# matt-graham/mici

Hardware: NVIDIA H100
Metric: leapfrog steps/sec (aggregate over chains) (higher is better)
Workload: dtype f64

## Files before the change

mici_b200/csrc/leapfrog_dmma.cuh:

```cuda
#pragma once
#include <cfloat>
#include <type_traits>

#include "targets.cuh"

namespace mb200 {

__device__ __forceinline__ void dmma_m8n8k4(double& c0, double& c1, double a, double b) {
  asm volatile(
      "mma.sync.aligned.m8n8k4.row.col.f64.f64.f64.f64 {%0,%1}, {%2}, {%3}, {%0,%1};\n"
      : "+d"(c0), "+d"(c1)
      : "d"(a), "d"(b));
}

__device__ __forceinline__ void dmma_m16n8k16(double& c0, double& c1, double& c2, double& c3,
                                              const double2 (&a)[2][2], const double2 (&b)[2]) {
  asm volatile(
      "mma.sync.aligned.m16n8k16.row.col.f64.f64.f64.f64 {%0,%1,%2,%3}, "
      "{%4,%5,%6,%7,%8,%9,%10,%11}, {%12,%13,%14,%15}, {%0,%1,%2,%3};\n"
      : "+d"(c0), "+d"(c1), "+d"(c2), "+d"(c3)
      : "d"(a[0][0].x), "d"(a[1][0].x), "d"(a[0][0].y), "d"(a[1][0].y),
        "d"(a[0][1].x), "d"(a[1][1].x), "d"(a[0][1].y), "d"(a[1][1].y),
        "d"(b[0].x), "d"(b[0].y), "d"(b[1].x), "d"(b[1].y));
}

__device__ __forceinline__ uint32_t smem_u32(const void* p) {
  return static_cast<uint32_t>(__cvta_generic_to_shared(p));
}

__device__ __forceinline__ void named_barrier_sync(int id, int nthreads) {
  asm volatile("bar.sync %0, %1;" ::"r"(id), "r"(nthreads) : "memory");
}

#ifndef MB200_K1_TRACE
#define MB200_K1_TRACE(phase)
#endif
#ifndef MB200_K1_TRACE_AFTER
#define MB200_K1_TRACE_AFTER(phase, x)
#endif
#ifndef MB200_K1_MARK
#define MB200_K1_MARK(id)
#endif

constexpr int DMMA_TILES_PER_CTA = 8;
#ifndef MB200_DMMA_GROUPS
#define MB200_DMMA_GROUPS 4
#endif
constexpr int DMMA_GROUPS = MB200_DMMA_GROUPS;
__host__ __device__ constexpr int dmma_tile_count(int g) {
  return DMMA_TILES_PER_CTA / DMMA_GROUPS + (g < DMMA_TILES_PER_CTA % DMMA_GROUPS ? 1 : 0);
}
__host__ __device__ constexpr int dmma_tile_start(int g) {
  return g * (DMMA_TILES_PER_CTA / DMMA_GROUPS) +
         (g < DMMA_TILES_PER_CTA % DMMA_GROUPS ? g : DMMA_TILES_PER_CTA % DMMA_GROUPS);
}
constexpr int DMMA_MAX_MT = (DMMA_TILES_PER_CTA + DMMA_GROUPS - 1) / DMMA_GROUPS;
constexpr int DMMA_THREADS = 32 * 4 * DMMA_GROUPS;
constexpr int DMMA_ROWS_PER_CTA = 8 * DMMA_TILES_PER_CTA;

template <int DP>
struct DmmaSmem {
  static constexpr int LDA = DP + 8;
  double A[DP * LDA];
  double P[DMMA_ROWS_PER_CTA * LDA];
  double psum[DMMA_ROWS_PER_CTA][4];
  double rscal[DMMA_ROWS_PER_CTA];
  double ex[2][DMMA_ROWS_PER_CTA][4];
  unsigned long long mbar;
};

template <class Target, int DP, int MT, bool PC>
__device__ __forceinline__ void leapfrog_dmma_group(
    DmmaSmem<DP>& sm, const Target& target, const double* q_in, const double* p_in,
    double* q_out, double* p_out, const int32_t* __restrict__ dir,
    const double* __restrict__ step_sizes, int64_t n_chains, int dim,
    double step_size, int n_steps, double* __restrict__ h_out, int32_t* __restrict__ status,
    int32_t* __restrict__ n_done, int64_t chain0, int row0, int w, int lane, int bar_id,
    int cta_threads, bool vec2, int32_t* __restrict__ counters) {
  constexpr int LDA = DmmaSmem<DP>::LDA;
  constexpr int NT = DP / 32;
  constexpr int KS = DP / 4;
  const int r = lane >> 2, c = lane & 3;
  const int col0 = w * (DP / 4);
  const double mh = -0.5 * step_size;
  const bool owner = (w == 0) && (c == 0);

  double q[MT][NT][2], mhr[PC ? MT : 1];
  bool live[MT];
  int row[MT];
  auto load_scale = [&](int64_t ch) {
    const double d = (dir != nullptr && dir[ch] < 0) ? -1.0 : 1.0;
    return PC ? d * step_sizes[ch] : d;
  };
  const uint32_t pofs = (uint32_t)((row0 + r) * LDA + col0 + 2 * c);
  auto pslot = [&](int mt, int nt) -> double2& {
    return *reinterpret_cast<double2*>(&sm.P[pofs + mt * 8 * LDA + 8 * nt]);
  };

#pragma unroll
  for (int mt = 0; mt < MT; ++mt) {
    row[mt] = row0 + 8 * mt + r;
    const int64_t ch = chain0 + row[mt];
    live[mt] = ch < n_chains;
    const double sgn = live[mt] ? load_scale(ch) : (PC ? 0.0 : 1.0);
    if (PC) mhr[mt] = -0.5 * (sgn * sgn);
#pragma unroll
    for (int nt = 0; nt < NT; ++nt) {
      const int i = col0 + 8 * nt + 2 * c;
      double2 a = make_double2(0.0, 0.0), b = make_double2(0.0, 0.0);
      if (live[mt] && i < dim) {
        if (vec2) {
          a = *reinterpret_cast<const double2*>(q_in + (size_t)ch * dim + i);
          b = *reinterpret_cast<const double2*>(p_in + (size_t)ch * dim + i);
        } else {
          a.x = q_in[(size_t)ch * dim + i], b.x = p_in[(size_t)ch * dim + i];
          if (i + 1 < dim) a.y = q_in[(size_t)ch * dim + i + 1], b.y = p_in[(size_t)ch * dim + i + 1];
        }
      }
      q[mt][nt][0] = a.x, q[mt][nt][1] = a.y;
      pslot(mt, nt) = make_double2(sgn * b.x, sgn * b.y);
    }
  }

  int s = -1;

  auto tile_sums = [&]() {
    if (!Target::TILE_SUM) return;
    double v[MT];
#pragma unroll
    for (int mt = 0; mt < MT; ++mt) {
      double t0 = q[mt][0][0] * q[mt][0][0];
      if (Target::COORD0) t0 = owner ? 0.0 : t0;
      t0 = fma(q[mt][0][1], q[mt][0][1], t0);
      if (mt == 0) MB200_K1_TRACE_AFTER(6, t0);
      double t1 = 0.0;
#pragma unroll
      for (int nt = 1; nt < NT; ++nt) {
        double& t = (nt & 1) ? t1 : t0;
        t = fma(q[mt][nt][0], q[mt][nt][0], t);
        t = fma(q[mt][nt][1], q[mt][nt][1], t);
      }
      v[mt] = t0 + t1;
    }
#pragma unroll
    for (int mt = 0; mt < MT; ++mt) v[mt] += __shfl_xor_sync(FULL_MASK, v[mt], 1);
#pragma unroll
    for (int mt = 0; mt < MT; ++mt) v[mt] += __shfl_xor_sync(FULL_MASK, v[mt], 2);
#pragma unroll
    for (int mt = 0; mt < MT; ++mt)
      if (c == 0) sm.psum[row[mt]][w] = v[mt];
  };
  auto publish_partials = [&]() {
    if (Target::ROW_SCALAR && w == 0) {
      double v0 = (c == 0) ? q[0][0][0] : 0.0;
#pragma unroll
      for (int mt = 1; mt < MT; ++mt) {
        const double vm = __shfl_sync(FULL_MASK, q[mt][0][0], lane & ~3);
        v0 = (c == mt) ? vm : v0;
      }
      tile_sums();
      const double rs = target.row_scalar(v0);
      if (c < MT) sm.rscal[row0 + 8 * c + r] = rs;
    } else {
      tile_sums();
    }
  };

  auto update_phase = [&](auto kicks_tag) {
    constexpr int KICKS = decltype(kicks_tag)::value;
    double2 pv[MT][NT];
    if (KICKS > 0) {
#pragma unroll
      for (int mt = 0; mt < MT; ++mt)
#pragma unroll
        for (int nt = 0; nt < NT; ++nt) pv[mt][nt] = pslot(mt, nt);
    }
    publish_partials();
    MB200_K1_TRACE(2);
    named_barrier_sync(bar_id, 128);
    MB200_K1_TRACE(3);
    if (KICKS == 0) return;
    double rs[MT];
#pragma unroll
    for (int mt = 0; mt < MT; ++mt) rs[mt] = Target::ROW_SCALAR ? sm.rscal[row[mt]] : 1.0;
#pragma unroll
    for (int mt = 0; mt < MT; ++mt) {
      const double mhm = PC ? mhr[PC ? mt : 0] : mh;
      const double coef = target.kick_coef(mhm, rs[mt]);
      double c00 = coef, a00 = q[mt][0][0];
      if (Target::COORD0 && w == 0) {
        const double4 ps = *reinterpret_cast<const double4*>(&sm.psum[row[mt]][0]);
        const double g0 = target.grad0(q[mt][0][0], ((ps.x + ps.y) + ps.z) + ps.w, rs[mt]);
        c00 = owner ? mhm : coef;
        a00 = owner ? g0 : a00;
      }
#pragma unroll
      for (int nt = 0; nt < NT; ++nt) {
        double2 v = pv[mt][nt];
        if (Target::LINEAR) {
#pragma unroll
          for (int k = 0; k < KICKS; ++k) {
            v.x = (nt == 0) ? fma(c00, a00, v.x) : fma(coef, q[mt][nt][0], v.x);
            v.y = fma(coef, q[mt][nt][1], v.y);
          }
        } else {
#pragma unroll
          for (int k = 0; k < KICKS; ++k)
            target.kick_pair_nl(mhm, q[mt][nt][0], q[mt][nt][1], v.x, v.y);
        }
        pslot(mt, nt) = v;
      }
    }
    MB200_K1_TRACE(4);
    named_barrier_sync(bar_id, 128);
    MB200_K1_TRACE(5);
  };
  using K0 = std::integral_constant<int, 0>;
  using K1 = std::integral_constant<int, 1>;
  using K2 = std::integral_constant<int, 2>;

  auto drift = [&](double (&acc)[MT][NT][2]) {
    const double2* a_base = reinterpret_cast<const double2*>(&sm.P[(row0 + r) * LDA + 2 * c]);
    const double2* b_base = reinterpret_cast<const double2*>(&sm.A[(col0 + r) * LDA + 2 * c]);
    if constexpr (MT == 2) {
#pragma unroll 2
      for (int j = 0; j < KS / 4; ++j) {
        double2 a[2][2], b[NT][2];
#pragma unroll
        for (int mt = 0; mt < 2; ++mt)
#pragma unroll
          for (int h = 0; h < 2; ++h) a[mt][h] = a_base[mt * 4 * LDA + 4 * (2 * j + h)];
#pragma unroll
        for (int nt = 0; nt < NT; ++nt)
#pragma unroll
          for (int h = 0; h < 2; ++h) b[nt][h] = b_base[nt * 4 * LDA + 4 * (2 * j + h)];
#pragma unroll
        for (int nt = 0; nt < NT; ++nt)
          dmma_m16n8k16(acc[0][nt][0], acc[0][nt][1], acc[1][nt][0], acc[1][nt][1], a, b[nt]);
      }
    } else {
      constexpr bool KSPLIT = (MT == 1);
      double acc2[KSPLIT ? NT : 1][2];
      if (KSPLIT) {
#pragma unroll
        for (int nt = 0; nt < NT; ++nt) acc2[nt][0] = 0.0, acc2[nt][1] = 0.0;
      }
#pragma unroll 4
      for (int j = 0; j < KS / 2; ++j) {
        double2 a[MT], b[NT];
#pragma unroll
        for (int mt = 0; mt < MT; ++mt) a[mt] = a_base[mt * 4 * LDA + 4 * j];
#pragma unroll
        for (int nt = 0; nt < NT; ++nt) b[nt] = b_base[nt * 4 * LDA + 4 * j];
#pragma unroll
        for (int mt = 0; mt < MT; ++mt)
#pragma unroll
          for (int nt = 0; nt < NT; ++nt)
            dmma_m8n8k4(acc[mt][nt][0], acc[mt][nt][1], a[mt].x, b[nt].x);
#pragma unroll
        for (int mt = 0; mt < MT; ++mt)
#pragma unroll
          for (int nt = 0; nt < NT; ++nt) {
            if (KSPLIT) dmma_m8n8k4(acc2[nt][0], acc2[nt][1], a[mt].y, b[nt].y);
            else dmma_m8n8k4(acc[mt][nt][0], acc[mt][nt][1], a[mt].y, b[nt].y);
          }
      }
      if (KSPLIT) {
#pragma unroll
        for (int nt = 0; nt < NT; ++nt) acc[0][nt][0] += acc2[nt][0], acc[0][nt][1] += acc2[nt][1];
      }
    }
  };

  MB200_K1_MARK(4);
  if (n_steps > 0) update_phase(K1{});
  else update_phase(K0{});
  MB200_K1_MARK(5);
  for (s = 0; s < n_steps - 1; ++s) {
    MB200_K1_TRACE(0);
    drift(q);
    MB200_K1_TRACE(1);
    update_phase(K2{});
  }
  if (n_steps > 0) {
    drift(q);
    update_phase(K1{});
  }

  MB200_K1_MARK(6);
#pragma unroll
  for (int mt = 0; mt < MT; ++mt) {
    const int64_t ch = chain0 + row[mt];
    if (!live[mt]) continue;
    const double sgn = load_scale(ch);
#pragma unroll
    for (int nt = 0; nt < NT; ++nt) {
      const int i = col0 + 8 * nt + 2 * c;
      if (i < dim) {
        const double2 sv = pslot(mt, nt);
        double2 pv = make_double2(sgn * sv.x, sgn * sv.y);
        if (PC) {
          if (sgn != 0.0) {
            pv = make_double2(sv.x / sgn, sv.y / sgn);
          } else {
            pv.x = p_in[(size_t)ch * dim + i];
            pv.y = (i + 1 < dim) ? p_in[(size_t)ch * dim + i + 1] : 0.0;
          }
          if (h_out != nullptr && !(sgn * sgn >= DBL_MIN)) pslot(mt, nt) = pv;
        }
        if (vec2) {
          *reinterpret_cast<double2*>(q_out + (size_t)ch * dim + i) =
              make_double2(q[mt][nt][0], q[mt][nt][1]);
          *reinterpret_cast<double2*>(p_out + (size_t)ch * dim + i) = pv;
        } else {
          q_out[(size_t)ch * dim + i] = q[mt][nt][0], p_out[(size_t)ch * dim + i] = pv.x;
          if (i + 1 < dim)
            q_out[(size_t)ch * dim + i + 1] = q[mt][nt][1], p_out[(size_t)ch * dim + i + 1] = pv.y;
        }
      }
    }
    if (w == 0 && c == 0) {
      if (status != nullptr) status[ch] = MB200_STATUS_OK;
      if (n_done != nullptr) n_done[ch] = n_steps;
      if (counters != nullptr) counters[ch * MB200_N_COUNTERS + MB200_COUNT_GRAD] += n_steps + 1;
    }
  }

  MB200_K1_MARK(7);
  if (h_out != nullptr) {
    if (PC) named_barrier_sync(bar_id, 128);
    double l[MT], kin[MT], u[MT][NT][2];
#pragma unroll
    for (int mt = 0; mt < MT; ++mt) {
      double red[2] = {0.0, 1.0};
      if (Target::TILE_SUM) {
        const double4 ps = *reinterpret_cast<const double4*>(&sm.psum[row[mt]][0]);
        red[0] = ((ps.x + ps.y) + ps.z) + ps.w;
      }
      if (Target::ROW_SCALAR) red[1] = sm.rscal[row[mt]];
      l[mt] = 0.0;
#pragma unroll
      for (int nt = 0; nt < NT; ++nt) {
        const int i = col0 + 8 * nt + 2 * c;
        if (i < dim) l[mt] += target.nld_pair(i, q[mt][nt][0], q[mt][nt][1], red);
        u[mt][nt][0] = 0.0, u[mt][nt][1] = 0.0;
      }
    }
    drift(u);
#pragma unroll
    for (int mt = 0; mt < MT; ++mt) {
      kin[mt] = 0.0;
#pragma unroll
      for (int nt = 0; nt < NT; ++nt) {
        const double2 sv = pslot(mt, nt);
        kin[mt] = fma(sv.x, u[mt][nt][0], kin[mt]);
        kin[mt] = fma(sv.y, u[mt][nt][1], kin[mt]);
      }
      kin[mt] += __shfl_xor_sync(FULL_MASK, kin[mt], 1);
      kin[mt] += __shfl_xor_sync(FULL_MASK, kin[mt], 2);
      l[mt] += __shfl_xor_sync(FULL_MASK, l[mt], 1);
      l[mt] += __shfl_xor_sync(FULL_MASK, l[mt], 2);
      if (c == 0) {
        sm.ex[0][row[mt]][w] = kin[mt];
        sm.ex[1][row[mt]][w] = l[mt];
      }
    }
    named_barrier_sync(bar_id, 128);
    if (w == 0 && c == 0) {
#pragma unroll
      for (int mt = 0; mt < MT; ++mt) {
        if (!live[mt]) continue;
        const double4 k4 = *reinterpret_cast<const double4*>(&sm.ex[0][row[mt]][0]);
        const double4 l4 = *reinterpret_cast<const double4*>(&sm.ex[1][row[mt]][0]);
        const double ks = ((k4.x + k4.y) + k4.z) + k4.w;
        const double ls = ((l4.x + l4.y) + l4.z) + l4.w;
        if (PC) {
          const double e = step_sizes[chain0 + row[mt]];
          h_out[chain0 + row[mt]] = ls + 0.5 * (e * e >= DBL_MIN ? ks / (e * e) : ks);
        } else {
          h_out[chain0 + row[mt]] = ls + 0.5 * (ks / step_size);
        }
      }
    }
  }
}

template <class Target, int DP, bool PC>
__global__ void __launch_bounds__(DMMA_THREADS, 1)
    leapfrog_dmma_kernel(const double* q_in, const double* p_in, double* q_out, double* p_out,
                         const int32_t* __restrict__ dir, const double* __restrict__ step_sizes,
                         int64_t n_chains, int dim,
                         double step_size, int n_steps, const double* __restrict__ minv,
                         ModelArgs model, double* __restrict__ h_out,
                         int32_t* __restrict__ status, int32_t* __restrict__ n_done,
                         int tiles_per_cta, int vec2, int tma_rows) {
  extern __shared__ __align__(128) unsigned char smem_raw[];
  DmmaSmem<DP>& sm = *reinterpret_cast<DmmaSmem<DP>*>(smem_raw);
  constexpr int LDA = DmmaSmem<DP>::LDA;
  const int tid = threadIdx.x;
  const int lane = tid & 31;
  const int warp = tid >> 5;
  const int group = warp >> 2;
  const int w = ((warp & 3) + group) & 3;
  const Target target(model, dim);
  MB200_K1_MARK(0);

  const uint32_t mbar = smem_u32(&sm.mbar);
  if (tma_rows && warp == 0) {
    if (lane == 0) {
      asm volatile("mbarrier.init.shared::cta.b64 [%0], 1;" ::"r"(mbar));
      asm volatile("fence.mbarrier_init.release.cluster;" ::: "memory");
    }
    __syncwarp();
    const uint32_t row_bytes = (uint32_t)dim * 8u;
    if (lane == 0)
      asm volatile("mbarrier.arrive.expect_tx.shared::cta.b64 _, [%0], %1;" ::"r"(mbar),
                   "r"(row_bytes * (uint32_t)dim)
                   : "memory");
    __syncwarp();
#pragma unroll 1
    for (int row = lane; row < dim; row += 32) {
      const unsigned long long src =
          reinterpret_cast<unsigned long long>(minv) + (unsigned long long)row * row_bytes;
      asm volatile(
          "cp.async.bulk.shared::cluster.global.mbarrier::complete_tx::bytes [%0], [%1], %2, [%3];"
          ::"r"(smem_u32(&sm.A[row * LDA])),
          "l"(src), "r"(row_bytes), "r"(mbar)
          : "memory");
    }
  }
  {
    const int64_t chain0 = (int64_t)blockIdx.x * (8 * tiles_per_cta);
    const int64_t left = n_chains - chain0;
    const int64_t rows = left < 8 * tiles_per_cta ? left : 8 * tiles_per_cta;
    const int64_t lines = (rows * dim * 8 + 127) / 128;
    for (int64_t i = tid; i < 2 * lines; i += blockDim.x) {
      const double* base = (i < lines ? q_in : p_in) + (size_t)chain0 * dim;
      const char* ptr = reinterpret_cast<const char*>(base) + (i < lines ? i : i - lines) * 128;
      asm volatile("prefetch.global.L2 [%0];" ::"l"(ptr));
    }
  }
  if (!tma_rows) {
    for (int idx = tid; idx < dim * dim; idx += blockDim.x) {
      const int row = idx / dim, col = idx - row * dim;
      sm.A[row * LDA + col] = minv[idx];
    }
  }
  if (dim < DP) {
    for (int idx = tid; idx < DP * DP; idx += blockDim.x) {
      const int row = idx / DP, col = idx - row * DP;
      if (row >= dim || col >= dim) sm.A[row * LDA + col] = 0.0;
    }
  }
  MB200_K1_MARK(1);
  __syncthreads();
  if (tma_rows) {
    uint32_t done = 0;
    while (!done) {
      asm volatile(
          "{\n .reg .pred p;\n mbarrier.try_wait.parity.shared::cta.b64 p, [%1], 0;\n"
          " selp.u32 %0, 1, 0, p;\n}"
          : "=r"(done)
          : "r"(mbar)
          : "memory");
    }
  }
  MB200_K1_MARK(2);
  if (!PC)
#pragma unroll 4
  for (int idx = tid; idx < DP * (DP / 2); idx += blockDim.x) {
    const int row = idx / (DP / 2), c2 = idx - row * (DP / 2);
    double2* ptr = reinterpret_cast<double2*>(&sm.A[row * LDA]) + c2;
    double2 v = *ptr;
    v.x *= step_size, v.y *= step_size;
    *ptr = v;
  }
  __syncthreads();
  MB200_K1_MARK(3);

  const int rows_per_cta = 8 * tiles_per_cta;
  for (int64_t blk = blockIdx.x; blk * rows_per_cta < n_chains; blk += gridDim.x) {
    const int64_t chain0 = blk * rows_per_cta;
    const int64_t left = n_chains - chain0;
    const int tiles = (int)((left >= rows_per_cta) ? tiles_per_cta : (left + 7) / 8);
    const int base = tiles / DMMA_GROUPS, rem = tiles % DMMA_GROUPS;
    const int mt = base + (group < rem ? 1 : 0);
    const int row0 = 8 * (group * base + (group < rem ? group : rem));
    const int cta_threads = 128 * (tiles < DMMA_GROUPS ? tiles : DMMA_GROUPS);
#define MB200_GROUP(MT)                                                                       \
  leapfrog_dmma_group<Target, DP, MT, PC>(sm, target, q_in, p_in, q_out, p_out, dir,          \
                                          step_sizes, n_chains, dim, step_size, n_steps,      \
                                          h_out, status, n_done, chain0, row0, w, lane,       \
                                          1 + group, cta_threads, vec2 != 0, model.counters)
    if (DMMA_MAX_MT >= 4 && mt == 4) MB200_GROUP(4);
    else if (DMMA_MAX_MT >= 3 && mt == 3) MB200_GROUP(3);
    else if (mt == 2) MB200_GROUP(2);
    else if (mt == 1) MB200_GROUP(1);
#undef MB200_GROUP
    __syncthreads();
  }
}

}
```

Measured before the change: 1.443 billion.

## Split each DMMA row group across two warps with register-held momenta and pairwise barriers

Each row group now uses two warps, each owning half of the columns, instead of four warps owning quarters. Momenta stay in registers, and a warp's own half feeds the tensor-core drift directly. Only the half the partner needs is published to shared memory, signalled with bar.arrive and a per-warp named barrier. This removes the second barrier per step and lets each warp start on its own half while the partner is still publishing. It halves the CTA thread count and raises the register load per thread, which may cut occupancy and latency hiding.

```diff
diff --git a/mici_b200/csrc/leapfrog_dmma.cuh b/mici_b200/csrc/leapfrog_dmma.cuh
--- a/mici_b200/csrc/leapfrog_dmma.cuh
+++ b/mici_b200/csrc/leapfrog_dmma.cuh
@@ -32,6 +32,10 @@
   asm volatile("bar.sync %0, %1;" ::"r"(id), "r"(nthreads) : "memory");
 }
 
+__device__ __forceinline__ void named_barrier_arrive(int id, int nthreads) {
+  asm volatile("bar.arrive %0, %1;" ::"r"(id), "r"(nthreads) : "memory");
+}
+
 #ifndef MB200_K1_TRACE
 #define MB200_K1_TRACE(phase)
 #endif
@@ -43,19 +47,9 @@
 #endif
 
 constexpr int DMMA_TILES_PER_CTA = 8;
-#ifndef MB200_DMMA_GROUPS
-#define MB200_DMMA_GROUPS 4
-#endif
-constexpr int DMMA_GROUPS = MB200_DMMA_GROUPS;
-__host__ __device__ constexpr int dmma_tile_count(int g) {
-  return DMMA_TILES_PER_CTA / DMMA_GROUPS + (g < DMMA_TILES_PER_CTA % DMMA_GROUPS ? 1 : 0);
-}
-__host__ __device__ constexpr int dmma_tile_start(int g) {
-  return g * (DMMA_TILES_PER_CTA / DMMA_GROUPS) +
-         (g < DMMA_TILES_PER_CTA % DMMA_GROUPS ? g : DMMA_TILES_PER_CTA % DMMA_GROUPS);
-}
+constexpr int DMMA_GROUPS = 4;
 constexpr int DMMA_MAX_MT = (DMMA_TILES_PER_CTA + DMMA_GROUPS - 1) / DMMA_GROUPS;
-constexpr int DMMA_THREADS = 32 * 4 * DMMA_GROUPS;
+constexpr int DMMA_THREADS = 32 * 2 * DMMA_GROUPS;
 constexpr int DMMA_ROWS_PER_CTA = 8 * DMMA_TILES_PER_CTA;
 
 template <int DP>
@@ -75,17 +69,22 @@
     double* q_out, double* p_out, const int32_t* __restrict__ dir,
     const double* __restrict__ step_sizes, int64_t n_chains, int dim,
     double step_size, int n_steps, double* __restrict__ h_out, int32_t* __restrict__ status,
-    int32_t* __restrict__ n_done, int64_t chain0, int row0, int w, int lane, int bar_id,
-    int cta_threads, bool vec2, int32_t* __restrict__ counters) {
+    int32_t* __restrict__ n_done, int64_t chain0, int row0, int h, int lane, int group, bool vec2,
+    int32_t* __restrict__ counters) {
+  static_assert(MT == 1 || MT == 2, "a group owns one or two row tiles");
   constexpr int LDA = DmmaSmem<DP>::LDA;
-  constexpr int NT = DP / 32;
-  constexpr int KS = DP / 4;
+  constexpr int NT = DP / 16;
+  constexpr int NQ = NT / 2;
   const int r = lane >> 2, c = lane & 3;
-  const int col0 = w * (DP / 4);
+  const int col0 = h * (DP / 2);
+  const int bar_pair = 1 + group;
+  const int bar_own = 6 + 2 * group + h;
+  const int bar_partner = bar_own ^ 1;
   const double mh = -0.5 * step_size;
-  const bool owner = (w == 0) && (c == 0);
+  const bool owner = (h == 0) && (c == 0);
 
   double q[MT][NT][2], mhr[PC ? MT : 1];
+  double2 sv[MT][NT];
   bool live[MT];
   int row[MT];
   auto load_scale = [&](int64_t ch) {
@@ -118,7 +117,7 @@
         }
       }
       q[mt][nt][0] = a.x, q[mt][nt][1] = a.y;
-      pslot(mt, nt) = make_double2(sgn * b.x, sgn * b.y);
+      sv[mt][nt] = make_double2(sgn * b.x, sgn * b.y);
     }
   }
 
@@ -126,32 +125,40 @@
 
   auto tile_sums = [&]() {
     if (!Target::TILE_SUM) return;
-    double v[MT];
-#pragma unroll
-    for (int mt = 0; mt < MT; ++mt) {
-      double t0 = q[mt][0][0] * q[mt][0][0];
-      if (Target::COORD0) t0 = owner ? 0.0 : t0;
-      t0 = fma(q[mt][0][1], q[mt][0][1], t0);
-      if (mt == 0) MB200_K1_TRACE_AFTER(6, t0);
-      double t1 = 0.0;
-#pragma unroll
-      for (int nt = 1; nt < NT; ++nt) {
-        double& t = (nt & 1) ? t1 : t0;
-        t = fma(q[mt][nt][0], q[mt][nt][0], t);
-        t = fma(q[mt][nt][1], q[mt][nt][1], t);
-      }
-      v[mt] = t0 + t1;
-    }
-#pragma unroll
-    for (int mt = 0; mt < MT; ++mt) v[mt] += __shfl_xor_sync(FULL_MASK, v[mt], 1);
-#pragma unroll
-    for (int mt = 0; mt < MT; ++mt) v[mt] += __shfl_xor_sync(FULL_MASK, v[mt], 2);
+    double v[MT][2];
 #pragma unroll
     for (int mt = 0; mt < MT; ++mt)
-      if (c == 0) sm.psum[row[mt]][w] = v[mt];
+#pragma unroll
+      for (int qq = 0; qq < 2; ++qq) {
+        const int n0 = qq * NQ;
+        double t0 = q[mt][n0][0] * q[mt][n0][0];
+        if (Target::COORD0 && qq == 0) t0 = owner ? 0.0 : t0;
+        t0 = fma(q[mt][n0][1], q[mt][n0][1], t0);
+        if (mt == 0 && qq == 0) MB200_K1_TRACE_AFTER(6, t0);
+        double t1 = 0.0;
+#pragma unroll
+        for (int n = 1; n < NQ; ++n) {
+          double& t = (n & 1) ? t1 : t0;
+          t = fma(q[mt][n0 + n][0], q[mt][n0 + n][0], t);
+          t = fma(q[mt][n0 + n][1], q[mt][n0 + n][1], t);
+        }
+        v[mt][qq] = t0 + t1;
+      }
+#pragma unroll
+    for (int mt = 0; mt < MT; ++mt)
+#pragma unroll
+      for (int qq = 0; qq < 2; ++qq) v[mt][qq] += __shfl_xor_sync(FULL_MASK, v[mt][qq], 1);
+#pragma unroll
+    for (int mt = 0; mt < MT; ++mt)
+#pragma unroll
+      for (int qq = 0; qq < 2; ++qq) v[mt][qq] += __shfl_xor_sync(FULL_MASK, v[mt][qq], 2);
+#pragma unroll
+    for (int mt = 0; mt < MT; ++mt)
+      if (c == 0)
+        *reinterpret_cast<double2*>(&sm.psum[row[mt]][2 * h]) = make_double2(v[mt][0], v[mt][1]);
   };
   auto publish_partials = [&]() {
-    if (Target::ROW_SCALAR && w == 0) {
+    if (Target::ROW_SCALAR && h == 0) {
       double v0 = (c == 0) ? q[0][0][0] : 0.0;
 #pragma unroll
       for (int mt = 1; mt < MT; ++mt) {
@@ -166,125 +173,149 @@
     }
   };
 
-  auto update_phase = [&](auto kicks_tag) {
+  auto store_momenta = [&]() {
+#pragma unroll
+    for (int mt = 0; mt < MT; ++mt)
+#pragma unroll
+      for (int nt = 0; nt < NT; ++nt) pslot(mt, nt) = sv[mt][nt];
+    named_barrier_arrive(bar_own, 64);
+  };
+
+  auto update_phase = [&](auto kicks_tag, auto publish_tag) {
     constexpr int KICKS = decltype(kicks_tag)::value;
-    double2 pv[MT][NT];
-    if (KICKS > 0) {
-#pragma unroll
-      for (int mt = 0; mt < MT; ++mt)
-#pragma unroll
-        for (int nt = 0; nt < NT; ++nt) pv[mt][nt] = pslot(mt, nt);
-    }
+    constexpr bool PUBLISH = decltype(publish_tag)::value;
     publish_partials();
     MB200_K1_TRACE(2);
-    named_barrier_sync(bar_id, 128);
+    named_barrier_sync(bar_pair, 64);
     MB200_K1_TRACE(3);
-    if (KICKS == 0) return;
-    double rs[MT];
-#pragma unroll
-    for (int mt = 0; mt < MT; ++mt) rs[mt] = Target::ROW_SCALAR ? sm.rscal[row[mt]] : 1.0;
-#pragma unroll
-    for (int mt = 0; mt < MT; ++mt) {
-      const double mhm = PC ? mhr[PC ? mt : 0] : mh;
-      const double coef = target.kick_coef(mhm, rs[mt]);
-      double c00 = coef, a00 = q[mt][0][0];
-      if (Target::COORD0 && w == 0) {
-        const double4 ps = *reinterpret_cast<const double4*>(&sm.psum[row[mt]][0]);
-        const double g0 = target.grad0(q[mt][0][0], ((ps.x + ps.y) + ps.z) + ps.w, rs[mt]);
-        c00 = owner ? mhm : coef;
-        a00 = owner ? g0 : a00;
-      }
-#pragma unroll
-      for (int nt = 0; nt < NT; ++nt) {
-        double2 v = pv[mt][nt];
-        if (Target::LINEAR) {
-#pragma unroll
-          for (int k = 0; k < KICKS; ++k) {
-            v.x = (nt == 0) ? fma(c00, a00, v.x) : fma(coef, q[mt][nt][0], v.x);
-            v.y = fma(coef, q[mt][nt][1], v.y);
+    if (KICKS > 0) {
+      double rs[MT];
+#pragma unroll
+      for (int mt = 0; mt < MT; ++mt) rs[mt] = Target::ROW_SCALAR ? sm.rscal[row[mt]] : 1.0;
+#pragma unroll
+      for (int mt = 0; mt < MT; ++mt) {
+        const double mhm = PC ? mhr[PC ? mt : 0] : mh;
+        const double coef = target.kick_coef(mhm, rs[mt]);
+        double c00 = coef, a00 = q[mt][0][0];
+        if (Target::COORD0 && h == 0) {
+          const double4 ps = *reinterpret_cast<const double4*>(&sm.psum[row[mt]][0]);
+          const double g0 = target.grad0(q[mt][0][0], ((ps.x + ps.y) + ps.z) + ps.w, rs[mt]);
+          c00 = owner ? mhm : coef;
+          a00 = owner ? g0 : a00;
+        }
+#pragma unroll
+        for (int nt = 0; nt < NT; ++nt) {
+          double2 v = sv[mt][nt];
+          if (Target::LINEAR) {
+#pragma unroll
+            for (int k = 0; k < KICKS; ++k) {
+              v.x = (nt == 0) ? fma(c00, a00, v.x) : fma(coef, q[mt][nt][0], v.x);
+              v.y = fma(coef, q[mt][nt][1], v.y);
+            }
+          } else {
+#pragma unroll
+            for (int k = 0; k < KICKS; ++k)
+              target.kick_pair_nl(mhm, q[mt][nt][0], q[mt][nt][1], v.x, v.y);
           }
-        } else {
-#pragma unroll
-          for (int k = 0; k < KICKS; ++k)
-            target.kick_pair_nl(mhm, q[mt][nt][0], q[mt][nt][1], v.x, v.y);
-        }
-        pslot(mt, nt) = v;
+          sv[mt][nt] = v;
+        }
       }
     }
     MB200_K1_TRACE(4);
-    named_barrier_sync(bar_id, 128);
+    if (PUBLISH) store_momenta();
     MB200_K1_TRACE(5);
   };
   using K0 = std::integral_constant<int, 0>;
   using K1 = std::integral_constant<int, 1>;
   using K2 = std::integral_constant<int, 2>;
+  using Publish = std::true_type;
+  using Keep = std::false_type;
 
   auto drift = [&](double (&acc)[MT][NT][2]) {
-    const double2* a_base = reinterpret_cast<const double2*>(&sm.P[(row0 + r) * LDA + 2 * c]);
+    const int pcol0 = (h ^ 1) * (DP / 2);
+    const double2* a_base = reinterpret_cast<const double2*>(&sm.P[(row0 + r) * LDA + pcol0 + 2 * c]);
     const double2* b_base = reinterpret_cast<const double2*>(&sm.A[(col0 + r) * LDA + 2 * c]);
     if constexpr (MT == 2) {
-#pragma unroll 2
-      for (int j = 0; j < KS / 4; ++j) {
-        double2 a[2][2], b[NT][2];
-#pragma unroll
-        for (int mt = 0; mt < 2; ++mt)
-#pragma unroll
-          for (int h = 0; h < 2; ++h) a[mt][h] = a_base[mt * 4 * LDA + 4 * (2 * j + h)];
-#pragma unroll
-        for (int nt = 0; nt < NT; ++nt)
-#pragma unroll
-          for (int h = 0; h < 2; ++h) b[nt][h] = b_base[nt * 4 * LDA + 4 * (2 * j + h)];
-#pragma unroll
-        for (int nt = 0; nt < NT; ++nt)
-          dmma_m16n8k16(acc[0][nt][0], acc[0][nt][1], acc[1][nt][0], acc[1][nt][1], a, b[nt]);
-      }
+      auto kblock = [&](int k0, const double2 (&a)[2][2]) {
+#pragma unroll
+        for (int half = 0; half < 2; ++half) {
+          double2 b[NT / 2][2];
+#pragma unroll
+          for (int n = 0; n < NT / 2; ++n)
+#pragma unroll
+            for (int hh = 0; hh < 2; ++hh)
+              b[n][hh] = b_base[(half * NT / 2 + n) * 4 * LDA + (k0 + 8 * hh) / 2];
+#pragma unroll
+          for (int n = 0; n < NT / 2; ++n) {
+            const int nt = half * NT / 2 + n;
+            dmma_m16n8k16(acc[0][nt][0], acc[0][nt][1], acc[1][nt][0], acc[1][nt][1], a, b[n]);
+          }
+        }
+      };
+      auto own_half = [&]() {
+#pragma unroll
+        for (int j = 0; j < NT / 2; ++j) {
+          const double2 a[2][2] = {{sv[0][2 * j], sv[0][2 * j + 1]},
+                                   {sv[1][2 * j], sv[1][2 * j + 1]}};
+          kblock(col0 + 16 * j, a);
+        }
+      };
+      auto partner_half = [&]() {
+        named_barrier_sync(bar_partner, 64);
+#pragma unroll 1
+        for (int j = 0; j < NT / 2; ++j) {
+          double2 a[2][2];
+#pragma unroll
+          for (int mt = 0; mt < 2; ++mt)
+#pragma unroll
+            for (int hh = 0; hh < 2; ++hh) a[mt][hh] = a_base[mt * 4 * LDA + 4 * (2 * j + hh)];
+          kblock(pcol0 + 16 * j, a);
+        }
+      };
+      if (h == 0) own_half(), partner_half();
+      else partner_half(), own_half();
     } else {
-      constexpr bool KSPLIT = (MT == 1);
-      double acc2[KSPLIT ? NT : 1][2];
-      if (KSPLIT) {
-#pragma unroll
-        for (int nt = 0; nt < NT; ++nt) acc2[nt][0] = 0.0, acc2[nt][1] = 0.0;
-      }
-#pragma unroll 4
-      for (int j = 0; j < KS / 2; ++j) {
-        double2 a[MT], b[NT];
-#pragma unroll
-        for (int mt = 0; mt < MT; ++mt) a[mt] = a_base[mt * 4 * LDA + 4 * j];
-#pragma unroll
-        for (int nt = 0; nt < NT; ++nt) b[nt] = b_base[nt * 4 * LDA + 4 * j];
-#pragma unroll
-        for (int mt = 0; mt < MT; ++mt)
-#pragma unroll
-          for (int nt = 0; nt < NT; ++nt)
-            dmma_m8n8k4(acc[mt][nt][0], acc[mt][nt][1], a[mt].x, b[nt].x);
-#pragma unroll
-        for (int mt = 0; mt < MT; ++mt)
-#pragma unroll
-          for (int nt = 0; nt < NT; ++nt) {
-            if (KSPLIT) dmma_m8n8k4(acc2[nt][0], acc2[nt][1], a[mt].y, b[nt].y);
-            else dmma_m8n8k4(acc[mt][nt][0], acc[mt][nt][1], a[mt].y, b[nt].y);
-          }
-      }
-      if (KSPLIT) {
-#pragma unroll
-        for (int nt = 0; nt < NT; ++nt) acc[0][nt][0] += acc2[nt][0], acc[0][nt][1] += acc2[nt][1];
-      }
+      double acc2[NT][2];
+#pragma unroll
+      for (int nt = 0; nt < NT; ++nt) acc2[nt][0] = 0.0, acc2[nt][1] = 0.0;
+      auto kpair = [&](int k0, double2 a) {
+        double2 b[NT];
+#pragma unroll
+        for (int nt = 0; nt < NT; ++nt) b[nt] = b_base[nt * 4 * LDA + k0 / 2];
+#pragma unroll
+        for (int nt = 0; nt < NT; ++nt) dmma_m8n8k4(acc[0][nt][0], acc[0][nt][1], a.x, b[nt].x);
+#pragma unroll
+        for (int nt = 0; nt < NT; ++nt) dmma_m8n8k4(acc2[nt][0], acc2[nt][1], a.y, b[nt].y);
+      };
+      auto own_half = [&]() {
+#pragma unroll
+        for (int j = 0; j < NT; ++j) kpair(col0 + 8 * j, sv[0][j]);
+      };
+      auto partner_half = [&]() {
+        named_barrier_sync(bar_partner, 64);
+#pragma unroll 1
+        for (int j = 0; j < NT; ++j) kpair(pcol0 + 8 * j, a_base[4 * j]);
+      };
+      if (h == 0) own_half(), partner_half();
+      else partner_half(), own_half();
+#pragma unroll
+      for (int nt = 0; nt < NT; ++nt) acc[0][nt][0] += acc2[nt][0], acc[0][nt][1] += acc2[nt][1];
     }
   };
 
   MB200_K1_MARK(4);
-  if (n_steps > 0) update_phase(K1{});
-  else update_phase(K0{});
+  if (n_steps > 0) update_phase(K1{}, Publish{});
+  else update_phase(K0{}, Keep{});
   MB200_K1_MARK(5);
   for (s = 0; s < n_steps - 1; ++s) {
     MB200_K1_TRACE(0);
     drift(q);
     MB200_K1_TRACE(1);
-    update_phase(K2{});
+    update_phase(K2{}, Publish{});
   }
   if (n_steps > 0) {
     drift(q);
-    update_phase(K1{});
+    update_phase(K1{}, Keep{});
   }
 
   MB200_K1_MARK(6);
@@ -297,16 +328,16 @@
     for (int nt = 0; nt < NT; ++nt) {
       const int i = col0 + 8 * nt + 2 * c;
       if (i < dim) {
-        const double2 sv = pslot(mt, nt);
-        double2 pv = make_double2(sgn * sv.x, sgn * sv.y);
+        const double2 sm_v = sv[mt][nt];
+        double2 pv = make_double2(sgn * sm_v.x, sgn * sm_v.y);
         if (PC) {
           if (sgn != 0.0) {
-            pv = make_double2(sv.x / sgn, sv.y / sgn);
+            pv = make_double2(sm_v.x / sgn, sm_v.y / sgn);
           } else {
             pv.x = p_in[(size_t)ch * dim + i];
             pv.y = (i + 1 < dim) ? p_in[(size_t)ch * dim + i + 1] : 0.0;
           }
-          if (h_out != nullptr && !(sgn * sgn >= DBL_MIN)) pslot(mt, nt) = pv;
+          if (h_out != nullptr && !(sgn * sgn >= DBL_MIN)) sv[mt][nt] = pv;
         }
         if (vec2) {
           *reinterpret_cast<double2*>(q_out + (size_t)ch * dim + i) =
@@ -319,7 +350,7 @@
         }
       }
     }
-    if (w == 0 && c == 0) {
+    if (h == 0 && c == 0) {
       if (status != nullptr) status[ch] = MB200_STATUS_OK;
       if (n_done != nullptr) n_done[ch] = n_steps;
       if (counters != nullptr) counters[ch * MB200_N_COUNTERS + MB200_COUNT_GRAD] += n_steps + 1;
@@ -328,8 +359,8 @@
 
   MB200_K1_MARK(7);
   if (h_out != nullptr) {
-    if (PC) named_barrier_sync(bar_id, 128);
-    double l[MT], kin[MT], u[MT][NT][2];
+    store_momenta();
+    double l[MT][2], kin[MT][2], u[MT][NT][2];
 #pragma unroll
     for (int mt = 0; mt < MT; ++mt) {
       double red[2] = {0.0, 1.0};
@@ -338,35 +369,41 @@
         red[0] = ((ps.x + ps.y) + ps.z) + ps.w;
       }
       if (Target::ROW_SCALAR) red[1] = sm.rscal[row[mt]];
-      l[mt] = 0.0;
+      l[mt][0] = 0.0, l[mt][1] = 0.0;
 #pragma unroll
       for (int nt = 0; nt < NT; ++nt) {
         const int i = col0 + 8 * nt + 2 * c;
-        if (i < dim) l[mt] += target.nld_pair(i, q[mt][nt][0], q[mt][nt][1], red);
-        u[mt][nt][0] = 0.0, u[mt][nt][1] = 0.0;
-      }
-    }
+        if (i < dim) l[mt][nt / NQ] += target.nld_pair(i, q[mt][nt][0], q[mt][nt][1], red);
+      }
+    }
+#pragma unroll
+    for (int mt = 0; mt < MT; ++mt)
+#pragma unroll
+      for (int nt = 0; nt < NT; ++nt) u[mt][nt][0] = 0.0, u[mt][nt][1] = 0.0;
     drift(u);
 #pragma unroll
     for (int mt = 0; mt < MT; ++mt) {
-      kin[mt] = 0.0;
-#pragma unroll
-      for (int nt = 0; nt < NT; ++nt) {
-        const double2 sv = pslot(mt, nt);
-        kin[mt] = fma(sv.x, u[mt][nt][0], kin[mt]);
-        kin[mt] = fma(sv.y, u[mt][nt][1], kin[mt]);
-      }
-      kin[mt] += __shfl_xor_sync(FULL_MASK, kin[mt], 1);
-      kin[mt] += __shfl_xor_sync(FULL_MASK, kin[mt], 2);
-      l[mt] += __shfl_xor_sync(FULL_MASK, l[mt], 1);
-      l[mt] += __shfl_xor_sync(FULL_MASK, l[mt], 2);
+#pragma unroll
+      for (int qq = 0; qq < 2; ++qq) {
+        double& k = kin[mt][qq];
+        k = 0.0;
+#pragma unroll
+        for (int nt = qq * NQ; nt < (qq + 1) * NQ; ++nt) {
+          k = fma(sv[mt][nt].x, u[mt][nt][0], k);
+          k = fma(sv[mt][nt].y, u[mt][nt][1], k);
+        }
+        k += __shfl_xor_sync(FULL_MASK, k, 1);
+        k += __shfl_xor_sync(FULL_MASK, k, 2);
+        l[mt][qq] += __shfl_xor_sync(FULL_MASK, l[mt][qq], 1);
+        l[mt][qq] += __shfl_xor_sync(FULL_MASK, l[mt][qq], 2);
+      }
       if (c == 0) {
-        sm.ex[0][row[mt]][w] = kin[mt];
-        sm.ex[1][row[mt]][w] = l[mt];
-      }
-    }
-    named_barrier_sync(bar_id, 128);
-    if (w == 0 && c == 0) {
+        *reinterpret_cast<double2*>(&sm.ex[0][row[mt]][2 * h]) = make_double2(kin[mt][0], kin[mt][1]);
+        *reinterpret_cast<double2*>(&sm.ex[1][row[mt]][2 * h]) = make_double2(l[mt][0], l[mt][1]);
+      }
+    }
+    named_barrier_sync(bar_pair, 64);
+    if (h == 0 && c == 0) {
 #pragma unroll
       for (int mt = 0; mt < MT; ++mt) {
         if (!live[mt]) continue;
@@ -400,8 +437,8 @@
   const int tid = threadIdx.x;
   const int lane = tid & 31;
   const int warp = tid >> 5;
-  const int group = warp >> 2;
-  const int w = ((warp & 3) + group) & 3;
+  const int group = warp & 3;
+  const int h = warp >> 2;
   const Target target(model, dim);
   MB200_K1_MARK(0);
 
@@ -486,15 +523,13 @@
     const int base = tiles / DMMA_GROUPS, rem = tiles % DMMA_GROUPS;
     const int mt = base + (group < rem ? 1 : 0);
     const int row0 = 8 * (group * base + (group < rem ? group : rem));
-    const int cta_threads = 128 * (tiles < DMMA_GROUPS ? tiles : DMMA_GROUPS);
+    static_assert(DMMA_MAX_MT == 2, "a group owns at most two row tiles");
 #define MB200_GROUP(MT)                                                                       \
   leapfrog_dmma_group<Target, DP, MT, PC>(sm, target, q_in, p_in, q_out, p_out, dir,          \
                                           step_sizes, n_chains, dim, step_size, n_steps,      \
-                                          h_out, status, n_done, chain0, row0, w, lane,       \
-                                          1 + group, cta_threads, vec2 != 0, model.counters)
-    if (DMMA_MAX_MT >= 4 && mt == 4) MB200_GROUP(4);
-    else if (DMMA_MAX_MT >= 3 && mt == 3) MB200_GROUP(3);
-    else if (mt == 2) MB200_GROUP(2);
+                                          h_out, status, n_done, chain0, row0, h, lane,       \
+                                          group, vec2 != 0, model.counters)
+    if (mt == 2) MB200_GROUP(2);
     else if (mt == 1) MB200_GROUP(1);
 #undef MB200_GROUP
     __syncthreads();
```

Measured after the change: 1.493 billion (median of 6 runs). +3.5%, better.
